# LunaJang/Metabuli_work

Hardware: AMD Instinct MI355X
Metric: reads/sec classified (150bp & 10kb) vs GTDB-scale DB at 1/2/4/8 MI355X (higher is better)
Workload: dtype u64

## Files before the change

### metabuli_work_amd/csrc/mtb_assign.hip

```cpp
#include <algorithm>
#include <vector>

#include "mtb_launch.h"
#include "mtb_stdsort.h"

namespace mtb {

struct Path {
    int start, end;
    float score;
    int hd, depth;
    uint32_t sm, em;
};

__device__ __forceinline__ void match_key(const mtb_match& m, uint64_t& hi, uint64_t& lo) {
    hi = ((uint64_t)m.species_id << 32) | ((uint64_t)info_frame(m.qinfo) << 29) | (info_pos(m.qinfo) & 0x1FFFFFFFu);
    lo = ((uint64_t)m.hamming << 56) | ((uint64_t)(m.dna_encoding & 0xFFFFFFu) << 32) | m.target_id;
}

__device__ __forceinline__ bool key_gt(uint64_t ah, uint64_t al, uint64_t bh, uint64_t bl) {
    return ah > bh || (ah == bh && al > bl);
}

constexpr int kSmallSeg = 512;
// ... 2011 lines not shown
        const uint32_t reh = M[p.sm].right_end_hamming;
        p.start = c.end + 1;
        p.hd = max(0, p.hd - ham_fields(reh, range, true));
        p.score = p.score - score_fields(reh, range, true) - (float)(ol % 3);
    }
}

__device__ __forceinline__ void trim_path_reh(Path& p, const Path& c, int ol, uint32_t rehS, uint32_t rehE) {
    const int range = ol / 3;
    if (p.start < c.start) {
        p.end = c.start - 1;
        p.hd = max(0, p.hd - ham_fields(rehE, range, false));
        p.score = p.score - score_fields(rehE, range, false) - (float)(ol % 3);
    } else {
        p.start = c.end + 1;
        p.hd = max(0, p.hd - ham_fields(rehS, range, true));
        p.score = p.score - score_fields(rehS, range, true) - (float)(ol % 3);
    }
}

__device__ float combine_serial(const mtb_match* __restrict__ M, Path* Ps, long nP, Path* Cs) {
    stdsort::sort(Ps, Ps + nP, [](const Path& a, const Path& b) {
        if (a.score != b.score) return a.score > b.score;
        if (a.hd != b.hd) return a.hd < b.hd;
        return a.start > b.start;
    });
    long nC = 0;
    float score = 0.0f;
    for (long pi = 0; pi < nP; pi++) {
        if (nC == 0) {
            Cs[nC++] = Ps[pi];
            score += Ps[pi].score;
            continue;
        }
        bool overlapped = false;
        for (long j = 0; j < nC; j++) {
            Path& p = Ps[pi];
            const Path c = Cs[j];
            if ((p.end < c.start) || (c.end < p.start)) continue;
            const int ol = min(p.end, c.end) - max(p.start, c.start) + 1;
            if (ol == p.end - p.start + 1) { overlapped = true; break; }
            if (ol < 24) {
                trim_path(M, p, c, ol);
                continue;
            }
            overlapped = true;
            break;
        }
        if (!overlapped) {
            Cs[nC++] = Ps[pi];
            score += Ps[pi].score;
        }
    }
    return score;
}

__device__ __forceinline__ void species_score(float score, int readLength, const AssignCfg& cfg, float* spScore,
                                              uint8_t* spKeep, uint64_t s) {
    score = score / (float)readLength;
    score = (1.0f < score) ? 1.0f : score;
    spScore[s] = score;
    spKeep[s] = !(score < cfg.minScore);
}

constexpr int kWaveCombineMin = 24;
constexpr int kWaveCombineMax = 1024;

__global__ void __launch_bounds__(256) k_combine_paths(const mtb_match* __restrict__ M, const uint64_t* __restrict__ sStart,
                                                       uint64_t nS, const uint64_t* __restrict__ runGroup,
                                                       const uint64_t* __restrict__ gStart,
                                                       const uint32_t* __restrict__ pathCnt,
                                                       const uint32_t* __restrict__ qlen, AssignCfg cfg,
                                                       Path* __restrict__ P, Path* __restrict__ C,
                                                       float* __restrict__ spScore, uint8_t* __restrict__ spKeep,
                                                       uint64_t* __restrict__ waveList, uint32_t* __restrict__ waveCount) {
    const uint64_t s = (uint64_t)blockIdx.x * blockDim.x + threadIdx.x;
    if (s >= nS) return;
    const uint64_t ss = sStart[s], se = sStart[s + 1];
    uint64_t w = ss;
    for (uint64_t g = runGroup[s]; gStart[g] < se; g++) {
        const uint64_t src = gStart[g];
        const uint32_t cnt = pathCnt[g];
        if (src != w)
            for (uint32_t k = 0; k < cnt; k++) P[w + k] = P[src + k];
        w += cnt;
    }
    if (w == ss) { spKeep[s] = 0; return; }
    const long nP = (long)(w - ss);
    if (!cfg.generic && nP > kWaveCombineMin && nP <= kWaveCombineMax) {
        waveList[atomicAdd(waveCount, 1u)] = ((uint64_t)nP << 32) | s;
        return;
    }
    const int readLength = (int)qlen[info_seq(M[ss].qinfo) - 1];
    species_score(combine_serial(M, P + ss, nP, C + ss), readLength, cfg, spScore, spKeep, s);
}

__global__ void __launch_bounds__(64) k_combine_wave(const mtb_match* __restrict__ M, const uint64_t* __restrict__ sStart,
                                                     const uint64_t* __restrict__ waveList,
                                                     const uint32_t* __restrict__ qlen, AssignCfg cfg,
                                                     Path* __restrict__ P, Path* __restrict__ C,
                                                     float* __restrict__ spScore, uint8_t* __restrict__ spKeep,
                                                     unsigned long long* __restrict__ stats,
                                                     const uint64_t* __restrict__ order) {
    __shared__ uint64_t kbuf[2 * kWaveCombineMax];
    uint64_t* kh = kbuf;
    uint64_t* kl = kbuf + kWaveCombineMax;
    __shared__ uint16_t qrs[kWaveCombineMax], qre[kWaveCombineMax];
    const uint64_t e = waveList[order ? order[blockIdx.x] : blockIdx.x];
    const uint64_t s = (uint32_t)e;
    const int nP = (int)(e >> 32);
    const uint64_t ss = sStart[s];
    const Path* Ps = P + ss;
    const int lane = threadIdx.x;
    const int readLength = (int)qlen[info_seq(M[ss].qinfo) - 1];
    int p2 = 2;
    while (p2 < nP) p2 <<= 1;
    for (int i = lane; i < p2; i += 64) {
        if (i < nP) {
            const Path p = Ps[i];
            kh[i] = ((uint64_t)(~__float_as_uint(p.score)) << 32) | (uint32_t)p.hd;
            kl[i] = ((uint64_t)(~(uint32_t)p.start) << 32) | (uint32_t)i;
        } else {
            kh[i] = ~0ull;
            kl[i] = ~0ull;
        }
    }
    __syncthreads();
    for (int k = 2; k <= p2; k <<= 1) {
        for (int j = k >> 1; j > 0; j >>= 1) {
            for (int t = lane; t < (p2 >> 1); t += 64) {
                const int i = ((t & ~(j - 1)) << 1) | (t & (j - 1));
                const int ixj = i + j;
                const bool up = (i & k) == 0;
                const uint64_t ah = kh[i], al = kl[i], bh = kh[ixj], bl = kl[ixj];
                if (key_gt(ah, al, bh, bl) == up) {
                    kh[i] = bh; kl[i] = bl; kh[ixj] = ah; kl[ixj] = al;
                }
            }
            __syncthreads();
        }
    }
    bool tie = false;
    for (int i = lane; i + 1 < nP; i += 64) {
        if (kh[i] != kh[i + 1] || (kl[i] >> 32) != (kl[i + 1] >> 32)) continue;
        const Path a = Ps[(uint32_t)kl[i]], b = Ps[(uint32_t)kl[i + 1]];
        tie |= a.end != b.end || M[a.sm].right_end_hamming != M[b.sm].right_end_hamming ||
               M[a.em].right_end_hamming != M[b.em].right_end_hamming;
    }
    struct EmuKey {
        float score;
        int hd, start;
        uint32_t idx;
    };
    static_assert(sizeof(EmuKey) * kWaveCombineMax == sizeof(uint64_t) * 2 * kWaveCombineMax, "emulation keys fit");
    EmuKey* K = reinterpret_cast<EmuKey*>(kbuf);
    const bool emulate = __syncthreads_or(tie || cfg.emulateAll);
    if (emulate) {
        if (lane == 0) atomicAdd(&stats[1], 1ull);
        for (int i = lane; i < nP; i += 64) {
            const Path q = Ps[i];
            K[i] = EmuKey{q.score, q.hd, q.start, (uint32_t)i};
        }
        __syncthreads();
        if (lane == 0)
            stdsort::sort(K, K + nP, [](const EmuKey& a, const EmuKey& b) {
                if (a.score != b.score) return a.score > b.score;
                if (a.hd != b.hd) return a.hd < b.hd;
                return a.start > b.start;
            });
        __syncthreads();
    }
    constexpr int kPerLane = kWaveCombineMax / 64;
    uint32_t src[kPerLane];
#pragma unroll
    for (int t = 0; t < kPerLane; t++) {
        const int i = lane + 64 * t;
        src[t] = i < nP ? (emulate ? K[i].idx : (uint32_t)kl[i]) : 0u;
    }
    __syncthreads();
    int* qs = reinterpret_cast<int*>(kh);
    int* qe = qs + kWaveCombineMax;
    float* qsc = reinterpret_cast<float*>(kl);
    int* qhd = reinterpret_cast<int*>(kl) + kWaveCombineMax;
#pragma unroll
    for (int t = 0; t < kPerLane; t++) {
        const int i = lane + 64 * t;
        if (i < nP) {
            const Path q = Ps[src[t]];
            qs[i] = q.start; qe[i] = q.end; qsc[i] = q.score; qhd[i] = q.hd;
            qrs[i] = M[q.sm].right_end_hamming;
            qre[i] = M[q.em].right_end_hamming;
        }
    }
    __syncthreads();
    constexpr int kSlots = kWaveCombineMax / 64;
    int rs[kSlots], re[kSlots];
#pragma unroll
    for (int t = 0; t < kSlots; t++) { rs[t] = 0; re[t] = -1; }
    float score = 0.0f;
    int nC = 0;
    for (int pi = 0; pi < nP; pi++) {
        Path p;
        p.start = qs[pi]; p.end = qe[pi]; p.score = qsc[pi]; p.hd = qhd[pi]; p.sm = 0; p.em = 0;
        const uint32_t rehS = qrs[pi], rehE = qre[pi];
        p.depth = 0;
        bool keep = true;
#pragma unroll
        for (int t = 0; t < kSlots; t++) {
            if (!keep || 64 * t >= nC) break;
            unsigned long long m = __ballot(64 * t + lane < nC && !(p.end < rs[t] || re[t] < p.start));
            while (keep && m) {
                const int l = __ffsll((long long)m) - 1;
                m &= m - 1;
                Path c;
                c.start = __shfl(rs[t], l, 64);
                c.end = __shfl(re[t], l, 64);
                if ((p.end < c.start) || (c.end < p.start)) continue;
                const int ol = min(p.end, c.end) - max(p.start, c.start) + 1;
                if (ol == p.end - p.start + 1) { keep = false; break; }
                if (ol < 24) { trim_path_reh(p, c, ol, rehS, rehE); continue; }
                keep = false;
            }
        }
        if (keep) {
#pragma unroll
            for (int t = 0; t < kSlots; t++)
                if (t == (nC >> 6) && lane == (nC & 63)) { rs[t] = p.start; re[t] = p.end; }
            nC++;
            score += p.score;
        }
    }
    if (lane == 0) species_score(score, readLength, cfg, spScore, spKeep, s);
}

__device__ long filter_redundant_serial(const mtb_match* __restrict__ M, uint64_t bestFirst, uint64_t bestSecond,
                                        uint64_t bestGroup, const uint64_t* __restrict__ gStart,
                                        uint32_t dnaShift, const TaxView& tax, mtb_taxcnt* __restrict__ tc) {
    uint32_t fc[6], fin[6], head[6];
    const mtb_match* B = M + bestFirst;
    int nf = 0;
    for (uint64_t g = bestGroup; nf < 6 && gStart[g] < bestSecond; g++) {
        fc[nf] = (uint32_t)(gStart[g] - bestFirst);
        fin[nf] = (uint32_t)(gStart[g + 1] - bestFirst);
        nf++;
    }
#pragma unroll
    for (int f = 0; f < 6; f++) head[f] = (f < nf) ? info_pos(B[fc[f]].qinfo) / dnaShift : 0xFFFFFFFFu;
    constexpr int kRegTc = 4;
    int32_t rt[kRegTc];
    uint32_t rc[kRegTc];
    long nTc = 0;
    while (true) {
        uint32_t qmin = 0xFFFFFFFFu;
#pragma unroll
        for (int f = 0; f < 6; f++) qmin = min(qmin, head[f]);
        if (qmin == 0xFFFFFFFFu) break;
        uint32_t minH = 256;
        int32_t t = 0;
#pragma unroll
        for (int f = 0; f < 6; f++) {
            while (head[f] == qmin) {
                const mtb_match& x = B[fc[f]];
                const uint32_t h = x.hamming;
                if (h < minH) { minH = h; t = (int32_t)x.target_id; }
                else if (h == minH) t = tax.lca(t, (int32_t)x.target_id);
                fc[f]++;
                head[f] = fc[f] < fin[f] ? info_pos(B[fc[f]].qinfo) / dnaShift : 0xFFFFFFFFu;
            }
        }
        long e = -1;
#pragma unroll
        for (int k = 0; k < kRegTc; k++)
            if (k < nTc && rt[k] == t) e = k;
        if (e >= 0) {
#pragma unroll
            for (int k = 0; k < kRegTc; k++)
                if (k == e) rc[k]++;
            continue;
        }
        if (nTc < kRegTc) {
#pragma unroll
            for (int k = 0; k < kRegTc; k++)
                if (k == nTc) { rt[k] = t; rc[k] = 1; }
            nTc++;
            continue;
        }
        e = kRegTc;
        while (e < nTc && tc[e].tax_id != t) e++;
        if (e == nTc) { tc[nTc].tax_id = t; tc[nTc].count = 0; nTc++; }
        tc[e].count++;
    }
#pragma unroll
    for (int k = 0; k < kRegTc; k++)
        if (k < nTc) { tc[k].tax_id = rt[k]; tc[k].count = rc[k]; }
    for (long a = 1; a < nTc; a++) {
        mtb_taxcnt v = tc[a];
        long b = a;
        while (b > 0 && tc[b - 1].tax_id > v.tax_id) { tc[b] = tc[b - 1]; b--; }
        tc[b] = v;
    }
    return nTc;
}

__device__ void classify_tail(mtb_result& res, const mtb_taxcnt* __restrict__ tc, long nTc, float spTotal,
                              int32_t bestTax, int readLength, const AssignCfg& cfg, const TaxView& tax,
                              Clade* __restrict__ cl, long clCap) {
    res.taxcnt_offset = (uint32_t)0;
    res.taxcnt_len = (uint32_t)nTc;
    res.is_classified = 1;
    res.score = spTotal;
    if (spTotal < cfg.minSpScore) {
        res.classification = tax.exists(bestTax) ? tax.spParent[tax.nodeOf[bestTax]] : 0;
        return;
    }
    if (cfg.em) {
        res.classification = bestTax;
        return;
    }
    const int32_t spT = bestTax;
    long nCl = 0;
    auto findOrAdd = [&](int32_t t) -> long {
        for (long z = 0; z < nCl; z++)
            if (cl[z].tax == t) return z;
        if (nCl >= clCap) return -1;
        cl[nCl].tax = t;
        cl[nCl].parentTax = 0;
        cl[nCl].count = 0;
        cl[nCl].removed = 0;
        return nCl++;
    };
    for (long e = 0; e < nTc; e++) {
        const uint32_t c = tc[e].count;
        int node = tax.nodeOf[tc[e].tax_id];
        int32_t t = tax.nodeTax[node];
        long z = findOrAdd(t);
        if (z < 0) break;
        cl[z].count += c;
        int guard = 0;
        while (t != spT && guard++ < 64) {
            const int pnode = tax.parent[node];
            const int32_t pt = tax.nodeTax[pnode];
            cl[z].parentTax = pt;
            long pz = findOrAdd(pt);
            if (pz < 0) break;
            cl[pz].count += c;
            node = pnode;
            t = pt;
            z = pz;
        }
    }
    if (cfg.accessionLevel == 2) {
        for (long z = 0; z < nCl; z++)
            if (cl[z].tax != spT && (tax.flags[tax.nodeOf[cl[z].tax]] & 2u)) cl[z].removed = 1;
    }
    const uint32_t thr = (uint32_t)((readLength - 1) / cfg.denominator);
    int32_t cur = spT;
    for (int step = 0; step < 64; step++) {
        uint32_t maxCnt = thr;
        long nBest = 0, best = -1, nChild = 0;
        for (long z = 0; z < nCl; z++) {
            if (cl[z].tax == spT || cl[z].removed || cl[z].parentTax != cur) continue;
            nChild++;
            const uint32_t cc = cl[z].count;
            if (cc > maxCnt) { maxCnt = cc; best = z; nBest = 1; }
            else if (cc == maxCnt) { if (nBest == 0) best = z; nBest++; }
        }
        if (nChild == 0 || nBest != 1) break;
        cur = cl[best].tax;
    }
    res.classification = cur;
}

__device__ __forceinline__ mtb_result empty_result(int readLength) {
    mtb_result res;
    res.classification = 0;
    res.score = 0.0f;
    res.hamming_dist = 0;
    res.query_length = (uint32_t)readLength;
    res.taxcnt_offset = (uint32_t)0;
    res.taxcnt_len = 0;
    res.is_classified = 0;
    for (int k = 0; k < 7; k++) res.pad[k] = 0;
    return res;
}

__global__ void __launch_bounds__(256) k_choose_taxon(const mtb_match* __restrict__ M, const uint64_t* __restrict__ mOff,
                                                      const uint32_t* __restrict__ qlen, uint32_t nReads,
                                                      const uint64_t* __restrict__ runOff,
                                                      const uint64_t* __restrict__ sStart,
                                                      const uint64_t* __restrict__ runGroup,
                                                      const uint64_t* __restrict__ gStart,
                                                      const float* __restrict__ spScore,
                                                      const uint8_t* __restrict__ spKeep, AssignCfg cfg, TaxView tax,
                                                      Clade* __restrict__ cladeP,
                                                      uint32_t cladePerMatch, mtb_taxcnt* __restrict__ tcP,
                                                      mtb_result* __restrict__ results) {
    const uint32_t r = blockIdx.x * blockDim.x + threadIdx.x;
    if (r >= nReads) return;
    const uint64_t base = mOff[r];
    const long n = (long)(mOff[r + 1] - base);
    const int readLength = (int)qlen[r];
    mtb_result res = empty_result(readLength);
    if (n == 0) { results[r] = res; return; }

    const uint64_t s0 = runOff[r], s1 = runOff[r + 1];
    long meaningful = 0;
    float bestSpScore = 0.0f;
    uint64_t bestFirst = 0, bestSecond = 0, bestRun = 0;
    for (uint64_t s = s0; s < s1; s++) {
        if (!spKeep[s]) continue;
        const float score = spScore[s];
        if (score > 0.f) meaningful++;
        if (score > bestSpScore) { bestSpScore = score; bestFirst = sStart[s]; bestSecond = sStart[s + 1]; bestRun = s; }
    }

    float spTotal = 0.0f;
    int32_t bestTax = 0;
    bool isLCA = false;
    if (meaningful > 0) {
        const float thr = bestSpScore * cfg.tieRatio;
        long cnt = 0;
        int lcaNode = -1;
        for (uint64_t s = s0; s < s1; s++) {
            if (!spKeep[s]) continue;
            if (spScore[s] >= thr) {
                cnt++;
                spTotal += spScore[s];
                const int32_t t = (int32_t)M[sStart[s]].species_id;
                if (cnt == 1) bestTax = t;
                if (tax.exists(t)) lcaNode = lcaNode < 0 ? tax.nodeOf[t] : tax.lca_node(lcaNode, tax.nodeOf[t]);
            }
        }
        if (cnt > 1) {
            isLCA = true;
            bestTax = lcaNode >= 0 ? tax.nodeTax[lcaNode] : 0;
            spTotal = spTotal / (float)cnt;
        }
    }
    if (spTotal == 0 || spTotal < cfg.minScore) {
        res.score = spTotal;
        results[r] = res;
        return;
    }
    if (isLCA) {
        res.is_classified = 1;
        res.classification = bestTax;
        res.score = spTotal;
        results[r] = res;
        return;
    }
    mtb_taxcnt* tc = tcP + base;
    const long nTc = filter_redundant_serial(M, bestFirst, bestSecond, runGroup[bestRun], gStart, (uint32_t)cfg.dnaShift, tax, tc);
    classify_tail(res, tc, nTc, spTotal, bestTax, readLength, cfg, tax, cladeP + base * cladePerMatch,
                  n * (long)cladePerMatch);
    results[r] = res;
}

constexpr int kWavePerReadMatches = 256;
constexpr int kQuotLds = 4096;
constexpr int kTcHash = 256;

__device__ __forceinline__ float wave_max_f(float x) {
#pragma unroll
    for (int d = 32; d > 0; d >>= 1) x = fmaxf(x, __shfl_xor(x, d, 64));
    return x;
}
__device__ __forceinline__ long wave_sum_l(long x) {
#pragma unroll
    for (int d = 32; d > 0; d >>= 1) x += __shfl_xor(x, d, 64);
    return x;
}

__global__ void __launch_bounds__(64) k_choose_taxon_wave(const mtb_match* __restrict__ M, const uint64_t* __restrict__ mOff,
                                                          const uint32_t* __restrict__ qlen, uint32_t nReads,
                                                          const uint64_t* __restrict__ runOff,
                                                          const uint64_t* __restrict__ sStart,
                                                          const uint64_t* __restrict__ runGroup,
                                                          const uint64_t* __restrict__ gStart,
                                                          const float* __restrict__ spScore,
                                                          const uint8_t* __restrict__ spKeep, AssignCfg cfg,
                                                          TaxView tax, Clade* __restrict__ cladeP,
                                                          uint32_t cladePerMatch, mtb_taxcnt* __restrict__ tcP,
                                                          mtb_result* __restrict__ results,
                                                          const uint64_t* __restrict__ order) {
    __shared__ uint32_t qw[kQuotLds];
    __shared__ int32_t hk[kTcHash];
    __shared__ uint32_t hc[kTcHash];
    __shared__ int sFlag;
    if (blockIdx.x >= nReads) return;
    const uint32_t r = order ? (uint32_t)order[blockIdx.x] : blockIdx.x;
    const int lane = threadIdx.x;
    const uint64_t base = mOff[r];
    const long n = (long)(mOff[r + 1] - base);
    const int readLength = (int)qlen[r];
    mtb_result res = empty_result(readLength);
    if (n == 0) {
        if (lane == 0) results[r] = res;
        return;
    }
    const uint64_t s0 = runOff[r], s1 = runOff[r + 1];
    long meaningful = 0;
    float bestSpScore = 0.0f;
    for (uint64_t s = s0 + lane; s < s1; s += 64) {
        if (!spKeep[s]) continue;
        const float score = spScore[s];
        meaningful += score > 0.f;
        bestSpScore = fmaxf(bestSpScore, score);
    }
    meaningful = wave_sum_l(meaningful);
    bestSpScore = wave_max_f(bestSpScore);
    float spTotal = 0.0f;
    int32_t bestTax = 0;
    bool isLCA = false;
    uint64_t bestFirst = 0, bestSecond = 0, bestRun = 0;
    if (meaningful > 0) {
        for (uint64_t c = s0; c < s1; c += 64) {
            const uint64_t s = c + lane;
            const bool hit = s < s1 && spKeep[s] && spScore[s] == bestSpScore;
            const unsigned long long m = __ballot(hit);
            if (m) {
                const uint64_t sb = c + (uint64_t)(__ffsll((long long)m) - 1);
                bestRun = sb;
                bestFirst = sStart[sb];
                bestSecond = sStart[sb + 1];
                break;
            }
        }
        const float thr = bestSpScore * cfg.tieRatio;
        long cnt = 0;
        int lcaNode = -1;
        for (uint64_t c = s0; c < s1; c += 64) {
            const uint64_t s = c + lane;
            const bool in = s < s1 && spKeep[s] && spScore[s] >= thr;
            const float sc = in ? spScore[s] : 0.0f;
            const int32_t sp = in ? (int32_t)M[sStart[s]].species_id : 0;
            unsigned long long m = __ballot(in);
            while (m) {
                const int b = __ffsll((long long)m) - 1;
                m &= m - 1;
                const float v = __shfl(sc, b, 64);
                const int32_t t = __shfl(sp, b, 64);
                cnt++;
                spTotal += v;
                if (cnt == 1) bestTax = t;
                if (tax.exists(t)) lcaNode = lcaNode < 0 ? tax.nodeOf[t] : tax.lca_node(lcaNode, tax.nodeOf[t]);
            }
        }
        if (cnt > 1) {
            isLCA = true;
            bestTax = lcaNode >= 0 ? tax.nodeTax[lcaNode] : 0;
            spTotal = spTotal / (float)cnt;
        }
    }
    if (spTotal == 0 || spTotal < cfg.minScore || isLCA) {
        if (lane == 0) {
            res.score = spTotal;
            if (isLCA && !(spTotal == 0 || spTotal < cfg.minScore)) {
                res.is_classified = 1;
                res.classification = bestTax;
            }
            results[r] = res;
        }
        return;
    }
    mtb_taxcnt* tc = tcP + base;
    const uint32_t dnaShift = (uint32_t)cfg.dnaShift;
    const long maxQ = (readLength + 3) / (long)dnaShift;
    const long nb = (long)(bestSecond - bestFirst);
    const mtb_match* B = M + bestFirst;
    long nTc = -1;
    if (tax.maxTax < 0xFFFFFF) {
        for (int k = lane; k < kTcHash; k += 64) { hk[k] = 0; hc[k] = 0; }
        if (lane == 0) sFlag = 0;
        for (long q0 = 0; q0 <= maxQ; q0 += kQuotLds) {
            const long q1 = min(maxQ + 1, q0 + (long)kQuotLds);
            for (long q = q0 + lane; q < q1; q += 64) qw[q - q0] = 0xFFFFFFFFu;
            __syncthreads();
            for (long i = lane; i < nb; i += 64) {
                const uint32_t q = info_pos(B[i].qinfo) / dnaShift;
                if (q > (uint32_t)maxQ || B[i].hamming > 254u) { sFlag = 1; continue; }
                if ((long)q < q0 || (long)q >= q1) continue;
                atomicMin(&qw[q - q0], (uint32_t)B[i].hamming << 24 | 0xFFFFFFu);
            }
            __syncthreads();
            if (sFlag) break;
            for (long i = lane; i < nb; i += 64) {
                const uint32_t q = info_pos(B[i].qinfo) / dnaShift;
                if ((long)q < q0 || (long)q >= q1) continue;
                const uint32_t h = (uint32_t)B[i].hamming << 24;
                uint32_t old = qw[q - q0];
                if ((old & 0xFF000000u) != h) continue;
                const int32_t t = (int32_t)B[i].target_id;
                while (true) {
                    const uint32_t cur = old & 0xFFFFFFu;
                    const uint32_t nv = h | (uint32_t)(cur == 0xFFFFFFu ? t : tax.lca((int32_t)cur, t));
                    if (nv == old) break;
                    const uint32_t prev = atomicCAS(&qw[q - q0], old, nv);
                    if (prev == old) break;
                    old = prev;
                }
            }
            __syncthreads();
            for (long q = q0 + lane; q < q1; q += 64) {
                const uint32_t wq = qw[q - q0];
                const int32_t t = wq == 0xFFFFFFFFu ? 0 : (int32_t)(wq & 0xFFFFFFu);
                if (t == 0) continue;
                uint32_t h = ((uint32_t)t * 2654435761u) & (kTcHash - 1);
                int probes = 0;
                while (true) {
                    const int32_t prev = atomicCAS(&hk[h], 0, t);
                    if (prev == 0 || prev == t) { atomicAdd(&hc[h], 1u); break; }
                    h = (h + 1) & (kTcHash - 1);
                    if (++probes == kTcHash) { sFlag = 1; break; }
                }
            }
            __syncthreads();
            if (sFlag) break;
        }
        if (!sFlag) {
            long at = 0;
            for (int k0 = 0; k0 < kTcHash; k0 += 64) {
                const int k = k0 + lane;
                const bool v = hk[k] != 0;
                const unsigned long long m = __ballot(v);
                if (v) {
                    const long p = at + (long)__popcll(m & ((1ull << lane) - 1));
                    tc[p].tax_id = hk[k];
                    tc[p].count = hc[k];
                }
                at += (long)__popcll(m);
            }
            nTc = at;
        }
    }
    if (lane != 0) return;
    if (nTc < 0) {
        nTc = filter_redundant_serial(M, bestFirst, bestSecond, runGroup[bestRun], gStart, dnaShift, tax, tc);
    } else {
        for (long a = 1; a < nTc; a++) {
            mtb_taxcnt v = tc[a];
            long b = a;
            while (b > 0 && tc[b - 1].tax_id > v.tax_id) { tc[b] = tc[b - 1]; b--; }
            tc[b] = v;
        }
    }
    classify_tail(res, tc, nTc, spTotal, bestTax, readLength, cfg, tax, cladeP + base * cladePerMatch,
                  n * (long)cladePerMatch);
    results[r] = res;
}

constexpr int kGroupLanes = 16;
constexpr int kGroupQ = 128;
constexpr int kGroupHash = 64;

__device__ __forceinline__ float group_max_f(float x) {
#pragma unroll
    for (int d = kGroupLanes / 2; d > 0; d >>= 1) x = fmaxf(x, __shfl_xor(x, d, kGroupLanes));
    return x;
}
__device__ __forceinline__ long group_sum_l(long x) {
#pragma unroll
    for (int d = kGroupLanes / 2; d > 0; d >>= 1) x += __shfl_xor(x, d, kGroupLanes);
    return x;
}

__device__ __forceinline__ void group_lds_order() {
    __builtin_amdgcn_fence(__ATOMIC_RELEASE, "wavefront");
    __builtin_amdgcn_wave_barrier();
    __builtin_amdgcn_fence(__ATOMIC_ACQUIRE, "wavefront");
}

__global__ void __launch_bounds__(256) k_choose_taxon_group(const mtb_match* __restrict__ M,
                                                            const uint64_t* __restrict__ mOff,
                                                            const uint32_t* __restrict__ qlen, uint32_t nReads,
                                                            const uint64_t* __restrict__ runOff,
                                                            const uint64_t* __restrict__ sStart,
                                                            const uint64_t* __restrict__ runGroup,
                                                            const uint64_t* __restrict__ gStart,
                                                            const float* __restrict__ spScore,
                                                            const uint8_t* __restrict__ spKeep, AssignCfg cfg,
                                                            TaxView tax, Clade* __restrict__ cladeP,
                                                            uint32_t cladePerMatch, mtb_taxcnt* __restrict__ tcP,
                                                            mtb_result* __restrict__ results) {
    constexpr int kGroups = 256 / kGroupLanes;
    __shared__ uint32_t qw[kGroups][kGroupQ];
    __shared__ int32_t hk[kGroups][kGroupHash];
    __shared__ uint32_t hc[kGroups][kGroupHash];
    __shared__ int gFlag[kGroups];
    const int g = threadIdx.x / kGroupLanes, gl = threadIdx.x % kGroupLanes;
    const int gLane0 = (threadIdx.x & 63) & ~(kGroupLanes - 1);
    const uint32_t r = blockIdx.x * kGroups + g;
    const bool valid = r < nReads;
    const uint64_t base = valid ? mOff[r] : 0;
    const long n = valid ? (long)(mOff[r + 1] - base) : 0;
    const int readLength = valid ? (int)qlen[r] : 0;
    mtb_result res = empty_result(readLength);
    float spTotal = 0.0f;
    int32_t bestTax = 0;
    bool isLCA = false, filter = false;
    uint64_t bestFirst = 0, bestSecond = 0, bestRun = 0;
    if (n > 0) {
        const uint64_t s0 = runOff[r], s1 = runOff[r + 1];
        long meaningful = 0;
        float bestSpScore = 0.0f;
        for (uint64_t s = s0 + gl; s < s1; s += kGroupLanes) {
            if (!spKeep[s]) continue;
            const float score = spScore[s];
            meaningful += score > 0.f;
            bestSpScore = fmaxf(bestSpScore, score);
        }
        meaningful = group_sum_l(meaningful);
        bestSpScore = group_max_f(bestSpScore);
        if (meaningful > 0) {
            for (uint64_t c = s0; c < s1; c += kGroupLanes) {
                const uint64_t s = c + gl;
                const bool hit = s < s1 && spKeep[s] && spScore[s] == bestSpScore;
                const uint32_t m = (uint32_t)(__ballot(hit) >> gLane0) & 0xFFFFu;
                if (m) {
                    const uint64_t sb = c + (uint64_t)(__ffs((int)m) - 1);
                    bestRun = sb;
                bestFirst = sStart[sb];
                    bestSecond = sStart[sb + 1];
                    break;
                }
            }
            const float thr = bestSpScore * cfg.tieRatio;
            long cnt = 0;
            int lcaNode = -1;
            for (uint64_t c = s0; c < s1; c += kGroupLanes) {
                const uint64_t s = c + gl;
                const bool in = s < s1 && spKeep[s] && spScore[s] >= thr;
                const float sc = in ? spScore[s] : 0.0f;
                const int32_t sp = in ? (int32_t)M[sStart[s]].species_id : 0;
                uint32_t m = (uint32_t)(__ballot(in) >> gLane0) & 0xFFFFu;
                while (m) {
                    const int b = __ffs((int)m) - 1;
                    m &= m - 1;
                    const float v = __shfl(sc, b, kGroupLanes);
                    const int32_t t = __shfl(sp, b, kGroupLanes);
                    cnt++;
                    spTotal += v;
                    if (cnt == 1) bestTax = t;
                    if (tax.exists(t)) lcaNode = lcaNode < 0 ? tax.nodeOf[t] : tax.lca_node(lcaNode, tax.nodeOf[t]);
                }
            }
            if (cnt > 1) {
                isLCA = true;
                bestTax = lcaNode >= 0 ? tax.nodeTax[lcaNode] : 0;
                spTotal = spTotal / (float)cnt;
            }
        }
        filter = !(spTotal == 0 || spTotal < cfg.minScore || isLCA);
    }
    const uint32_t dnaShift = (uint32_t)cfg.dnaShift;
    const long maxQ = (readLength + 3) / (long)dnaShift;
    const long nb = (long)(bestSecond - bestFirst);
    const mtb_match* B = M + bestFirst;
    const bool lds = filter && maxQ < kGroupQ && tax.maxTax < 0xFFFFFF;
    if (lds) {
        for (long q = gl; q <= maxQ; q += kGroupLanes) qw[g][q] = 0xFFFFFFFFu;
        for (int k = gl; k < kGroupHash; k += kGroupLanes) {
            hk[g][k] = 0;
            hc[g][k] = 0;
        }
        if (gl == 0) gFlag[g] = 0;
    }
    group_lds_order();
    if (lds) {
        for (long i = gl; i < nb; i += kGroupLanes) {
            const uint32_t q = info_pos(B[i].qinfo) / dnaShift;
            if (q > (uint32_t)maxQ || B[i].hamming > 254u) {
                gFlag[g] = 1;
                continue;
            }
            atomicMin(&qw[g][q], (uint32_t)B[i].hamming << 24 | 0xFFFFFFu);
        }
    }
    group_lds_order();
    const bool ok = lds && !gFlag[g];
    if (ok) {
        for (long i = gl; i < nb; i += kGroupLanes) {
            const uint32_t q = info_pos(B[i].qinfo) / dnaShift;
            const uint32_t h = (uint32_t)B[i].hamming << 24;
            uint32_t old = qw[g][q];
            if ((old & 0xFF000000u) != h) continue;
            const int32_t t = (int32_t)B[i].target_id;
            while (true) {
                const uint32_t cur = old & 0xFFFFFFu;
                const uint32_t nv = h | (uint32_t)(cur == 0xFFFFFFu ? t : tax.lca((int32_t)cur, t));
                if (nv == old) break;
                const uint32_t prev = atomicCAS(&qw[g][q], old, nv);
                if (prev == old) break;
                old = prev;
            }
        }
    }
    group_lds_order();
    if (ok) {
        for (long q = gl; q <= maxQ; q += kGroupLanes) {
            const uint32_t wq = qw[g][q];
            const int32_t t = wq == 0xFFFFFFFFu ? 0 : (int32_t)(wq & 0xFFFFFFu);
            if (t == 0) continue;
            uint32_t h = ((uint32_t)t * 2654435761u) & (kGroupHash - 1);
            int probes = 0;
            while (true) {
                const int32_t prev = atomicCAS(&hk[g][h], 0, t);
                if (prev == 0 || prev == t) {
                    atomicAdd(&hc[g][h], 1u);
                    break;
                }
                h = (h + 1) & (kGroupHash - 1);
                if (++probes == kGroupHash) {
                    gFlag[g] = 1;
                    break;
                }
            }
        }
    }
    group_lds_order();
    mtb_taxcnt* tc = tcP + base;
    long nTc = -1;
    const bool packed = ok && !gFlag[g];
    if (packed) {
        static_assert(2 * kGroupHash <= kGroupQ, "the packed taxa fit the quotient table");
        long at = 0;
        for (int k0 = 0; k0 < kGroupHash; k0 += kGroupLanes) {
            const int k = k0 + gl;
            const bool v = hk[g][k] != 0;
            const uint32_t m = (uint32_t)(__ballot(v) >> gLane0) & 0xFFFFu;
            if (v) {
                const long p = at + (long)__popc(m & ((1u << gl) - 1));
                qw[g][2 * p] = (uint32_t)hk[g][k];
                qw[g][2 * p + 1] = hc[g][k];
            }
            at += (long)__popc(m);
        }
        nTc = at;
    }
    group_lds_order();
    if (packed) {
        for (long e = gl; e < nTc; e += kGroupLanes) {
            const int32_t t = (int32_t)qw[g][2 * e];
            long at = 0;
            for (long j = 0; j < nTc; j++) at += (int32_t)qw[g][2 * j] < t;
            tc[at].tax_id = t;
            tc[at].count = qw[g][2 * e + 1];
        }
    }
    if (gl != 0 || !valid) return;
    if (!filter) {
        res.score = spTotal;
        if (isLCA && n > 0 && !(spTotal == 0 || spTotal < cfg.minScore)) {
            res.is_classified = 1;
            res.classification = bestTax;
        }
        results[r] = res;
        return;
    }
    if (nTc < 0) nTc = filter_redundant_serial(M, bestFirst, bestSecond, runGroup[bestRun], gStart, dnaShift, tax, tc);
    classify_tail(res, tc, nTc, spTotal, bestTax, readLength, cfg, tax, cladeP + base * cladePerMatch,
                  n * (long)cladePerMatch);
    results[r] = res;
}

__global__ void k_wave_size_keys(const uint64_t* __restrict__ waveList, uint32_t n, uint64_t* __restrict__ keys) {
    const uint32_t i = blockIdx.x * blockDim.x + threadIdx.x;
    if (i < n) keys[i] = (uint64_t)(kWaveCombineMax - (uint32_t)(waveList[i] >> 32));
}
__global__ void k_read_size_keys(const uint64_t* __restrict__ mOff, uint32_t n, uint64_t* __restrict__ keys) {
    const uint32_t i = blockIdx.x * blockDim.x + threadIdx.x;
    if (i < n) keys[i] = 0xFFFFFFull - min<uint64_t>(mOff[i + 1] - mOff[i], 0xFFFFFFull);
}

static const uint64_t* longest_first(uint32_t n, int bits, const AssignScratch& s, hipStream_t st) {
    bool inB = false;
    radix_sort_pairs(s.ordKA, s.ordVA, s.ordKB, s.ordVB, n, 0, bits, false, true, s.radixCounts, s.radixOffs,
                     s.scanTmp, &inB, st);
    return inB ? s.ordVB : s.ordVA;
}

void launch_assign(const mtb_match* matches, const uint64_t* mOff, const uint32_t* qlen, uint32_t nReads, uint64_t nM, const AssignArgs& a, const TaxDevice& t, const AssignScratch& s,
                   mtb_taxcnt* tcPool, mtb_result* results, unsigned long long* devStats, uint64_t* hostStats,
                   hipStream_t st) {
    for (int i = 0; i < 4; i++) hostStats[i] = 0;
    if (nReads == 0) return;
    AssignCfg cfg{a.kmerFormat, a.dnaShift, a.maxCodonShift, a.denominator, a.minConsCnt, a.minConsCntEuk,
                  a.accessionLevel, a.minScore, a.minSpScore, a.tieRatio, a.generic, a.emulateAll, a.em};
    TaxView tv{t.nodeOf, t.nodeTax, t.parent, t.depth, t.flags, t.spParent, t.maxTax};
    exclusive_scan_u32(s.grpCnt, nReads, s.grpOff, s.scanTmp, st);
    exclusive_scan_u32(s.runCnt, nReads, s.runOff, s.scanTmp, st);
    if (nM) {
        launch_run_starts(s.runFlag, mOff, s.grpOff, s.runOff, nReads, s.gStart, s.sStart, s.runGroup, st);
        uint64_t cnt[2] = {0, 0};
        hipMemcpyAsync(&cnt[0], s.grpOff + nReads, sizeof(uint64_t), hipMemcpyDeviceToHost, st);
        hipMemcpyAsync(&cnt[1], s.runOff + nReads, sizeof(uint64_t), hipMemcpyDeviceToHost, st);
        hipStreamSynchronize(st);
        hostStats[0] = cnt[0];
        hostStats[2] = cnt[1];
        if (cnt[0]) {
            k_group_keys<<<(unsigned)((cnt[0] + 255) / 256), 256, 0, st>>>(
                s.gStart, cnt[0], s.ordKA, s.ordVA, s.pathCnt,
                prune_min_matches(a.minConsCnt, a.minConsCntEuk, a.maxCodonShift));
            bool inB = false;
            const uint64_t heavy = radix_sort_pairs(s.ordKA, s.ordVA, s.ordKB, s.ordVB, cnt[0], 32, 40, true, false,
                                                    s.radixCounts, s.radixOffs, s.scanTmp, &inB, st);
            hostStats[1] = heavy;
            if (heavy) {
                const bool waves = !a.generic && a.bigGroups && nM >= kBigGroup;
                if (waves) hipMemsetAsync(s.waveCount, 0, sizeof(uint32_t), st);
                const char* nl = getenv("MTB_PATHS_NOLDS");
                const bool noLds = nl && atoi(nl) == 4;
                const char* la = getenv("MTB_K6_LOOKAHEAD");
                const bool look = !la || atoi(la) != 0;
#define MTB_PATHS(L, W, A)                                                                                          \
    k_match_paths<L, W, A><<<(unsigned)((heavy + 63) / 64), 64, 0, st>>>(                                              \
        matches, s.gStart, inB ? s.ordKB : s.ordKA, heavy, cfg, tv, (Path*)s.local, (Path*)s.paths, s.conn,         \
        s.pathCnt, waves ? s.waveList : nullptr, s.waveCount)
                if (noLds && look) MTB_PATHS(false, 4, true);
                else if (noLds) MTB_PATHS(false, 4, false);
                else if (look) MTB_PATHS(true, 1, true);
                else MTB_PATHS(true, 1, false);
#undef MTB_PATHS
                if (waves) {
                    uint32_t nBig = 0;
                    hipMemcpyAsync(&nBig, s.waveCount, sizeof(uint32_t), hipMemcpyDeviceToHost, st);
                    hipStreamSynchronize(st);
                    if (nBig && look)
                        k_match_paths_wave<true><<<nBig, 64, 0, st>>>(matches, s.gStart, s.waveList, cfg, tv, (Path*)s.local,
                                                                      (Path*)s.paths, s.conn, s.pathCnt);
                    else if (nBig)
                        k_match_paths_wave<false><<<nBig, 64, 0, st>>>(matches, s.gStart, s.waveList, cfg, tv, (Path*)s.local,
                                                                       (Path*)s.paths, s.conn, s.pathCnt);
                }
            }
        }
        if (cnt[1]) {
            hipMemsetAsync(s.waveCount, 0, sizeof(uint32_t), st);
            k_combine_paths<<<(unsigned)((cnt[1] + 255) / 256), 256, 0, st>>>(
                matches, s.sStart, cnt[1], s.runGroup, s.gStart, s.pathCnt, qlen, cfg, (Path*)s.paths, (Path*)s.comb,
                s.spScore, s.spKeep, s.waveList, s.waveCount);
            uint32_t nWave = 0;
            hipMemcpyAsync(&nWave, s.waveCount, sizeof(uint32_t), hipMemcpyDeviceToHost, st);
            hipStreamSynchronize(st);
            if (nWave) {
                k_wave_size_keys<<<(nWave + 255) / 256, 256, 0, st>>>(s.waveList, nWave, s.ordKA);
                const uint64_t* order = longest_first(nWave, 16, s, st);
                k_combine_wave<<<nWave, 64, 0, st>>>(matches, s.sStart, s.waveList, qlen, cfg, (Path*)s.paths,
                                                     (Path*)s.comb, s.spScore, s.spKeep, devStats, order);
            }
            hostStats[3] = nWave;
        }
    }
    const bool wave = a.waveTaxon >= 0 ? a.waveTaxon == 1 : (!a.generic && nM > (uint64_t)kWavePerReadMatches * nReads);
    const bool group = a.waveTaxon == 2 || (a.waveTaxon < 0 && !wave && !a.generic);
    if (group) {
        k_choose_taxon_group<<<(nReads + 15) / 16, 256, 0, st>>>(matches, mOff, qlen, nReads, s.runOff, s.sStart,
                                                                 s.runGroup, s.gStart, s.spScore, s.spKeep, cfg, tv,
                                                                 (Clade*)s.clade, s.cladePerMatch, tcPool, results);
    } else if (wave) {
        k_read_size_keys<<<(nReads + 255) / 256, 256, 0, st>>>(mOff, nReads, s.ordKA);
        const uint64_t* order = longest_first(nReads, 24, s, st);
        k_choose_taxon_wave<<<nReads, 64, 0, st>>>(matches, mOff, qlen, nReads, s.runOff, s.sStart, s.runGroup, s.gStart,
                                                   s.spScore, s.spKeep, cfg, tv, (Clade*)s.clade, s.cladePerMatch,
                                                   tcPool, results, order);
    } else {
        const unsigned ctT = nReads < 256u * 256u ? 64u : 256u;
        k_choose_taxon<<<(nReads + ctT - 1) / ctT, ctT, 0, st>>>(matches, mOff, qlen, nReads, s.runOff, s.sStart,
                                                             s.runGroup, s.gStart, s.spScore, s.spKeep, cfg, tv,
                                                             (Clade*)s.clade, s.cladePerMatch, tcPool, results);
    }
}

uint64_t path_bytes() { return sizeof(Path); }
uint64_t clade_bytes() { return sizeof(Clade); }

__global__ void k_compact_taxcnt(const mtb_taxcnt* __restrict__ pool, const uint64_t* __restrict__ mOff,
                                 mtb_result* __restrict__ results, const uint64_t* __restrict__ tcOff, uint32_t nReads,
                                 mtb_taxcnt* __restrict__ out) {
    uint32_t r = blockIdx.x * blockDim.x + threadIdx.x;
    if (r >= nReads) return;
    uint32_t len = results[r].taxcnt_len;
    uint64_t dst = tcOff[r];
    results[r].taxcnt_offset = (uint32_t)dst;
    for (uint32_t k = 0; k < len; k++) out[dst + k] = pool[mOff[r] + k];
}

__global__ void k_taxcnt_len(const mtb_result* __restrict__ results, uint32_t nReads, uint32_t* __restrict__ len) {
    uint32_t r = blockIdx.x * blockDim.x + threadIdx.x;
    if (r < nReads) len[r] = results[r].taxcnt_len;
}

void launch_taxcnt_len(const mtb_result* results, uint32_t nReads, uint32_t* len, hipStream_t s) {
    if (nReads) k_taxcnt_len<<<(nReads + 255) / 256, 256, 0, s>>>(results, nReads, len);
}
void launch_compact_taxcnt(const mtb_taxcnt* pool, const uint64_t* mOff, mtb_result* results, const uint64_t* tcOff,
                           uint32_t nReads, mtb_taxcnt* out, hipStream_t s) {
    if (nReads) k_compact_taxcnt<<<(nReads + 255) / 256, 256, 0, s>>>(pool, mOff, results, tcOff, nReads, out);
}

__global__ void k_chunk_totals(const uint32_t* __restrict__ cnt, uint32_t nChunks, uint32_t n,
                               uint32_t* __restrict__ tot) {
    const uint32_t r = blockIdx.x * blockDim.x + threadIdx.x;
    if (r >= n) return;
    uint32_t t = 0;
    for (uint32_t c = 0; c < nChunks; c++) t += cnt[(uint64_t)c * n + r];
    tot[r] = t;
}

__global__ void __launch_bounds__(256) k_regroup_chunks(const uint64_t* __restrict__ src, const uint32_t* __restrict__ cnt,
                                                        const uint64_t* __restrict__ srcOff, uint32_t nChunks, uint32_t n,
                                                        const uint64_t* __restrict__ mOff, uint64_t* __restrict__ dst) {
    const uint32_t r = blockIdx.x * 4 + threadIdx.x / 64;
    const uint32_t lane = threadIdx.x & 63;
    if (r >= n) return;
    uint64_t at = mOff[r] * 3;
    for (uint32_t c = 0; c < nChunks; c++) {
        const uint64_t k = (uint64_t)c * n + r;
        const uint64_t words = (uint64_t)cnt[k] * 3, from = srcOff[k] * 3;
        for (uint64_t w = lane; w < words; w += 64) dst[at + w] = src[from + w];
        at += words;
    }
}

void launch_regroup_chunks(const mtb_match* src, const uint32_t* cnt, uint32_t nChunks, uint32_t n, uint32_t* tot,
                           uint64_t* srcOff, uint64_t* mOff, void* scanTmp, mtb_match* dst, hipStream_t s) {
    if (!n) return;
    k_chunk_totals<<<(n + 255) / 256, 256, 0, s>>>(cnt, nChunks, n, tot);
    exclusive_scan_u32(tot, n, mOff, scanTmp, s);
    exclusive_scan_u32(cnt, (uint64_t)nChunks * n, srcOff, scanTmp, s);
    k_regroup_chunks<<<(n + 3) / 4, 256, 0, s>>>((const uint64_t*)src, cnt, srcOff, nChunks, n, mOff, (uint64_t*)dst);
}

struct EmPair {
    int32_t sp;
    float sc;
};

__global__ void k_em_top(const mtb_match* __restrict__ M, const uint64_t* __restrict__ mOff, uint32_t n,
                         const uint64_t* __restrict__ runOff, const uint64_t* __restrict__ sStart,
                         const float* __restrict__ spScore, const uint8_t* __restrict__ spKeep,
                         const mtb_result* __restrict__ results, EmPair* __restrict__ scratch,
                         EmPair* __restrict__ maps, uint8_t* __restrict__ cnt) {
    const uint32_t r = blockIdx.x * blockDim.x + threadIdx.x;
    if (r >= n) return;
    cnt[r] = 0;
    if (!results[r].is_classified) return;
    const uint64_t s0 = runOff[r], s1 = runOff[r + 1];
    EmPair* v = scratch + s0;
    long k = 0;
    for (uint64_t s = s0; s < s1; s++)
        if (spKeep[s]) v[k++] = EmPair{(int32_t)M[sStart[s]].species_id, spScore[s]};
    stdsort::sort(v, v + k, [](const EmPair& a, const EmPair& b) { return a.sc > b.sc; });
    const long m = k < kEmTop ? k : kEmTop;
    for (long i = 0; i < m; i++) maps[(uint64_t)r * kEmTop + i] = EmPair{v[i].sp, v[i].sc * v[i].sc};
    cnt[r] = (uint8_t)m;
}

void launch_em_top(const mtb_match* M, const uint64_t* mOff, uint32_t n, const AssignScratch& s,
                   const mtb_result* results, void* scratch, void* maps, uint8_t* cnt, hipStream_t st) {
    if (!n) return;
    k_em_top<<<(n + 255) / 256, 256, 0, st>>>(M, mOff, n, s.runOff, s.sStart, s.spScore, s.spKeep, results,
                                              (EmPair*)scratch, (EmPair*)maps, cnt);
}

__global__ void k_em_pack(const EmPair* __restrict__ maps, const uint8_t* __restrict__ cnt,
                          const uint64_t* __restrict__ off, uint32_t n, mtb_em_map* __restrict__ out) {
    const uint32_t r = blockIdx.x * blockDim.x + threadIdx.x;
    if (r >= n) return;
    const uint64_t o = off[r];
    for (uint32_t k = 0; k < cnt[r]; k++) {
        const EmPair e = maps[(uint64_t)r * kEmTop + k];
        out[o + k] = mtb_em_map{r, e.sp, e.sc};
    }
}

__global__ void k_u8_to_u32(const uint8_t* __restrict__ in, uint32_t n, uint32_t* __restrict__ out) {
    const uint32_t i = blockIdx.x * blockDim.x + threadIdx.x;
    if (i < n) out[i] = in[i];
}

void launch_em_pack(const void* maps, const uint8_t* cnt, uint32_t n, uint32_t* cnt32, uint64_t* off, void* scanTmp,
                    mtb_em_map* out, hipStream_t s) {
    if (!n) return;
    k_u8_to_u32<<<(n + 255) / 256, 256, 0, s>>>(cnt, n, cnt32);
    exclusive_scan_u32(cnt32, n, off, scanTmp, s);
    k_em_pack<<<(n + 255) / 256, 256, 0, s>>>((const EmPair*)maps, cnt, off, n, out);
}

__global__ void k_species_kmers(const DbRec* __restrict__ db, uint64_t D, const int32_t* __restrict__ spOf,
                                uint32_t maxTax, uint32_t* __restrict__ cnt) {
    MTB_GRID_STRIDE(i, D) {
        const uint32_t t = db[i].tax;
        const int32_t sp = t <= maxTax ? spOf[t] : 0;
        if (sp > 0) atomicAdd(&cnt[sp], 1u);
    }
}

void launch_species_kmers(const DbRec* db, uint64_t D, const int32_t* spOf, uint32_t maxTax, uint32_t* cnt,
                          hipStream_t s) {
    if (D) k_species_kmers<<<stride_grid(D), 256, 0, s>>>(db, D, spOf, maxTax, cnt);
}

__global__ void k_em_estep(const float* __restrict__ score, const uint32_t* __restrict__ spIdx,
                           const uint64_t* __restrict__ qOff, uint64_t nQ, const uint64_t* __restrict__ pos,
                           const double* __restrict__ p, const double* __restrict__ lf, double* __restrict__ wS,
                           unsigned long long* __restrict__ qCount) {
    const uint64_t q = (uint64_t)blockIdx.x * blockDim.x + threadIdx.x;
    bool counted = false;
    if (q < nQ) {
        const uint64_t a = qOff[q], b = qOff[q + 1];
        double denom = 0.0;
        for (uint64_t j = a; j < b; j++) denom += (double)score[j] * p[spIdx[j]] * lf[spIdx[j]];
        counted = !(denom == 0.0);
        for (uint64_t j = a; j < b; j++)
            wS[pos[j]] = counted ? ((double)score[j] * p[spIdx[j]] * lf[spIdx[j]]) / denom : 0.0;
    }
    const int c = __syncthreads_count(counted);
    if (threadIdx.x == 0 && c) atomicAdd(qCount, (unsigned long long)c);
}

__global__ void k_em_slices(const double* __restrict__ wS, const uint64_t* __restrict__ sliceOff, uint64_t nSl,
                            double* __restrict__ part) {
    const uint64_t i = (uint64_t)blockIdx.x * blockDim.x + threadIdx.x;
    if (i >= nSl) return;
    double f = 0.0;
    for (uint64_t j = sliceOff[i]; j < sliceOff[i + 1]; j++) f += wS[j];
    part[i] = f;
}

__global__ void k_em_mstep(const double* __restrict__ part, const uint64_t* __restrict__ spSlice, uint32_t S,
                           const uint8_t* __restrict__ isTop, const unsigned long long* __restrict__ qCount,
                           const double* __restrict__ p, double* __restrict__ pNew, double* __restrict__ absd,
                           int afterTen) {
    const uint32_t i = blockIdx.x * blockDim.x + threadIdx.x;
    if (i >= S) return;
    double f = 0.0;
    for (uint64_t k = spSlice[i]; k < spSlice[i + 1]; k++) f += part[k];
    if (isTop[i]) {
        f /= (double)*qCount;
        absd[i] = fabs(f - p[i]);
        if (afterTen && f < 1e-5) f = 0.0;
    } else {
        absd[i] = 0.0;
    }
    pNew[i] = f;
}

__global__ void __launch_bounds__(256) k_em_delta(const double* __restrict__ absd, uint32_t S, double* __restrict__ out) {
    __shared__ double part[256];
    const uint32_t per = (S + 255) / 256, a = threadIdx.x * per, b = min(S, a + per);
    double d = 0.0;
    for (uint32_t i = a; i < b; i++) d += absd[i];
    part[threadIdx.x] = d;
    __syncthreads();
    if (threadIdx.x == 0) {
        double t = 0.0;
        for (int k = 0; k < 256; k++) t += part[k];
        *out = t;
    }
}

void launch_em_iteration(const float* score, const uint32_t* spIdx, const uint64_t* qOff, uint64_t nQ,
                         const uint64_t* pos, const double* p, const double* lf, double* wS,
                         unsigned long long* qCount, const uint64_t* sliceOff, uint64_t nSl, double* part,
// ... 92 lines not shown
```

Measured before the change: 35.45 million.

## Keep clade table, sorted taxon counts and match fields on-chip in group assign

The group-per-read assign kernel now runs the clade-walk classification tail against a small LDS table that reuses the hash arrays. It falls back to the global clade buffer only when that table overflows, and reads the sorted taxon-count list from LDS when it is small. It also holds the first few match records per lane in registers between the min-hamming and LCA-fold passes, and caches per-lane species keep/score values when a read has at most one lane-stride of runs. The aim is to cut repeated global memory traffic in the serial lane-0 tail and the match re-reads, at the cost of extra registers, an extra wave barrier and a possible rerun when the table overflows.

```diff
diff --git a/metabuli_work_amd/csrc/mtb_assign.hip b/metabuli_work_amd/csrc/mtb_assign.hip
--- a/metabuli_work_amd/csrc/mtb_assign.hip
+++ b/metabuli_work_amd/csrc/mtb_assign.hip
@@ -2337,48 +2337,89 @@
     return nTc;
 }
 
-__device__ void classify_tail(mtb_result& res, const mtb_taxcnt* __restrict__ tc, long nTc, float spTotal,
-                              int32_t bestTax, int readLength, const AssignCfg& cfg, const TaxView& tax,
-                              Clade* __restrict__ cl, long clCap) {
+constexpr int kCladeLds = 32;
+struct TcGlobal {
+    const mtb_taxcnt* __restrict__ tc;
+    __device__ __forceinline__ int32_t tax(long e) const { return tc[e].tax_id; }
+    __device__ __forceinline__ uint32_t count(long e) const { return tc[e].count; }
+};
+struct TcLds {
+    const uint32_t* w;
+    __device__ __forceinline__ int32_t tax(long e) const { return (int32_t)w[2 * e]; }
+    __device__ __forceinline__ uint32_t count(long e) const { return w[2 * e + 1]; }
+};
+struct CladeGlobal {
+    static constexpr bool kRerun = false;
+    Clade* __restrict__ cl;
+    long cap;
+    __device__ __forceinline__ long capacity() const { return cap; }
+    __device__ __forceinline__ int32_t& tax(long z) const { return cl[z].tax; }
+    __device__ __forceinline__ int32_t& parentTax(long z) const { return cl[z].parentTax; }
+    __device__ __forceinline__ uint32_t& count(long z) const { return cl[z].count; }
+    __device__ __forceinline__ int32_t& removed(long z) const { return cl[z].removed; }
+};
+struct CladeLds {
+    static constexpr bool kRerun = true;
+    int32_t* k;
+    uint32_t* c;
+    long cap;
+    __device__ __forceinline__ long capacity() const { return cap; }
+    __device__ __forceinline__ int32_t& tax(long z) const { return k[z]; }
+    __device__ __forceinline__ int32_t& parentTax(long z) const { return k[kCladeLds + z]; }
+    __device__ __forceinline__ uint32_t& count(long z) const { return c[z]; }
+    __device__ __forceinline__ uint32_t& removed(long z) const { return c[kCladeLds + z]; }
+};
+
+template <typename Tc, typename Cl>
+__device__ __forceinline__ bool classify_tail_on(mtb_result& res, const Tc& tc, long nTc, float spTotal, int32_t bestTax,
+                                                 int readLength, const AssignCfg& cfg, const TaxView& tax,
+                                                 const Cl& cl) {
     res.taxcnt_offset = (uint32_t)0;
     res.taxcnt_len = (uint32_t)nTc;
     res.is_classified = 1;
     res.score = spTotal;
     if (spTotal < cfg.minSpScore) {
         res.classification = tax.exists(bestTax) ? tax.spParent[tax.nodeOf[bestTax]] : 0;
-        return;
+        return true;
     }
     if (cfg.em) {
         res.classification = bestTax;
-        return;
+        return true;
     }
     const int32_t spT = bestTax;
+    const long clCap = cl.capacity();
     long nCl = 0;
     auto findOrAdd = [&](int32_t t) -> long {
         for (long z = 0; z < nCl; z++)
-            if (cl[z].tax == t) return z;
+            if (cl.tax(z) == t) return z;
         if (nCl >= clCap) return -1;
-        cl[nCl].tax = t;
-        cl[nCl].parentTax = 0;
-        cl[nCl].count = 0;
-        cl[nCl].removed = 0;
+        cl.tax(nCl) = t;
+        cl.parentTax(nCl) = 0;
+        cl.count(nCl) = 0;
+        cl.removed(nCl) = 0;
         return nCl++;
     };
     for (long e = 0; e < nTc; e++) {
-        const uint32_t c = tc[e].count;
-        int node = tax.nodeOf[tc[e].tax_id];
+        const uint32_t c = tc.count(e);
+        int node = tax.nodeOf[tc.tax(e)];
         int32_t t = tax.nodeTax[node];
         long z = findOrAdd(t);
-        if (z < 0) break;
-        cl[z].count += c;
+        if (z < 0) {
+            if (Cl::kRerun) return false;
+            break;
+        }
+        cl.count(z) += c;
         int guard = 0;
         while (t != spT && guard++ < 64) {
             const int pnode = tax.parent[node];
             const int32_t pt = tax.nodeTax[pnode];
-            cl[z].parentTax = pt;
+            cl.parentTax(z) = pt;
             long pz = findOrAdd(pt);
-            if (pz < 0) break;
-            cl[pz].count += c;
+            if (pz < 0) {
+                if (Cl::kRerun) return false;
+                break;
+            }
+            cl.count(pz) += c;
             node = pnode;
             t = pt;
             z = pz;
@@ -2386,7 +2427,7 @@
     }
     if (cfg.accessionLevel == 2) {
         for (long z = 0; z < nCl; z++)
-            if (cl[z].tax != spT && (tax.flags[tax.nodeOf[cl[z].tax]] & 2u)) cl[z].removed = 1;
+            if (cl.tax(z) != spT && (tax.flags[tax.nodeOf[cl.tax(z)]] & 2u)) cl.removed(z) = 1;
     }
     const uint32_t thr = (uint32_t)((readLength - 1) / cfg.denominator);
     int32_t cur = spT;
@@ -2394,16 +2435,23 @@
         uint32_t maxCnt = thr;
         long nBest = 0, best = -1, nChild = 0;
         for (long z = 0; z < nCl; z++) {
-            if (cl[z].tax == spT || cl[z].removed || cl[z].parentTax != cur) continue;
+            if (cl.tax(z) == spT || cl.removed(z) || cl.parentTax(z) != cur) continue;
             nChild++;
-            const uint32_t cc = cl[z].count;
+            const uint32_t cc = cl.count(z);
             if (cc > maxCnt) { maxCnt = cc; best = z; nBest = 1; }
             else if (cc == maxCnt) { if (nBest == 0) best = z; nBest++; }
         }
         if (nChild == 0 || nBest != 1) break;
-        cur = cl[best].tax;
+        cur = cl.tax(best);
     }
     res.classification = cur;
+    return true;
+}
+
+__device__ void classify_tail(mtb_result& res, const mtb_taxcnt* __restrict__ tc, long nTc, float spTotal,
+                              int32_t bestTax, int readLength, const AssignCfg& cfg, const TaxView& tax,
+                              Clade* __restrict__ cl, long clCap) {
+    classify_tail_on(res, TcGlobal{tc}, nTc, spTotal, bestTax, readLength, cfg, tax, CladeGlobal{cl, clCap});
 }
 
 __device__ __forceinline__ mtb_result empty_result(int readLength) {
@@ -2687,6 +2735,10 @@
 constexpr int kGroupLanes = 16;
 constexpr int kGroupQ = 128;
 constexpr int kGroupHash = 64;
+constexpr int kHeld = 6;
+constexpr int kTcLds = 32;
+static_assert(2 * kCladeLds <= kGroupHash, "the on-chip clade table fits the two hash arrays");
+static_assert(4 * kTcLds <= kGroupQ, "packed pairs and sorted list fit the quotient table");
 
 __device__ __forceinline__ float group_max_f(float x) {
 #pragma unroll
@@ -2736,11 +2788,17 @@
     uint64_t bestFirst = 0, bestSecond = 0, bestRun = 0;
     if (n > 0) {
         const uint64_t s0 = runOff[r], s1 = runOff[r + 1];
+        const bool one = s1 - s0 <= (uint64_t)kGroupLanes;
+        const bool mine = one && s0 + gl < s1;
+        const uint8_t keepMine = mine ? spKeep[s0 + gl] : (uint8_t)0;
+        const float scoreMine = mine ? spScore[s0 + gl] : 0.0f;
+        auto kept = [&](uint64_t s) -> bool { return one ? keepMine != 0 : spKeep[s] != 0; };
+        auto scoreOf = [&](uint64_t s) -> float { return one ? scoreMine : spScore[s]; };
         long meaningful = 0;
         float bestSpScore = 0.0f;
         for (uint64_t s = s0 + gl; s < s1; s += kGroupLanes) {
-            if (!spKeep[s]) continue;
-            const float score = spScore[s];
+            if (!kept(s)) continue;
+            const float score = scoreOf(s);
             meaningful += score > 0.f;
             bestSpScore = fmaxf(bestSpScore, score);
         }
@@ -2749,12 +2807,12 @@
         if (meaningful > 0) {
             for (uint64_t c = s0; c < s1; c += kGroupLanes) {
                 const uint64_t s = c + gl;
-                const bool hit = s < s1 && spKeep[s] && spScore[s] == bestSpScore;
+                const bool hit = s < s1 && kept(s) && scoreOf(s) == bestSpScore;
                 const uint32_t m = (uint32_t)(__ballot(hit) >> gLane0) & 0xFFFFu;
                 if (m) {
                     const uint64_t sb = c + (uint64_t)(__ffs((int)m) - 1);
                     bestRun = sb;
-                bestFirst = sStart[sb];
+                    bestFirst = sStart[sb];
                     bestSecond = sStart[sb + 1];
                     break;
                 }
@@ -2764,8 +2822,8 @@
             int lcaNode = -1;
             for (uint64_t c = s0; c < s1; c += kGroupLanes) {
                 const uint64_t s = c + gl;
-                const bool in = s < s1 && spKeep[s] && spScore[s] >= thr;
-                const float sc = in ? spScore[s] : 0.0f;
+                const bool in = s < s1 && kept(s) && scoreOf(s) >= thr;
+                const float sc = in ? scoreOf(s) : 0.0f;
                 const int32_t sp = in ? (int32_t)M[sStart[s]].species_id : 0;
                 uint32_t m = (uint32_t)(__ballot(in) >> gLane0) & 0xFFFFu;
                 while (m) {
@@ -2801,34 +2859,59 @@
         if (gl == 0) gFlag[g] = 0;
     }
     group_lds_order();
-    if (lds) {
-        for (long i = gl; i < nb; i += kGroupLanes) {
-            const uint32_t q = info_pos(B[i].qinfo) / dnaShift;
-            if (q > (uint32_t)maxQ || B[i].hamming > 254u) {
-                gFlag[g] = 1;
-                continue;
-            }
-            atomicMin(&qw[g][q], (uint32_t)B[i].hamming << 24 | 0xFFFFFFu);
-        }
+    uint32_t heldQ[kHeld];
+    int32_t heldT[kHeld];
+    auto minHamming = [&](uint32_t q, uint32_t ham) -> bool {
+        if (q > (uint32_t)maxQ || ham > 254u) {
+            gFlag[g] = 1;
+            return false;
+        }
+        atomicMin(&qw[g][q], ham << 24 | 0xFFFFFFu);
+        return true;
+    };
+    auto foldTaxon = [&](uint32_t q, uint32_t h, int32_t t) {
+        uint32_t old = qw[g][q];
+        if ((old & 0xFF000000u) != h) return;
+        while (true) {
+            const uint32_t cur = old & 0xFFFFFFu;
+            const uint32_t nv = h | (uint32_t)(cur == 0xFFFFFFu ? t : tax.lca((int32_t)cur, t));
+            if (nv == old) break;
+            const uint32_t prev = atomicCAS(&qw[g][q], old, nv);
+            if (prev == old) break;
+            old = prev;
+        }
+    };
+#pragma unroll
+    for (int k = 0; k < kHeld; k++) {
+        heldQ[k] = 0xFFFFFFFFu;
+        heldT[k] = 0;
+    }
+    if (lds && nb > 0) {
+        uint32_t ham[kHeld];
+#pragma unroll
+        for (int k = 0; k < kHeld; k++) {
+            const long i = min((long)(gl + k * kGroupLanes), nb - 1);
+            heldQ[k] = info_pos(B[i].qinfo);
+            ham[k] = B[i].hamming;
+            heldT[k] = (int32_t)B[i].target_id;
+        }
+#pragma unroll
+        for (int k = 0; k < kHeld; k++) {
+            const uint32_t q = heldQ[k] / dnaShift;
+            const bool have = gl + k * kGroupLanes < nb;
+            heldQ[k] = have && minHamming(q, ham[k]) ? ham[k] << 24 | q : 0xFFFFFFFFu;
+        }
+        for (long i = gl + kHeld * kGroupLanes; i < nb; i += kGroupLanes)
+            minHamming(info_pos(B[i].qinfo) / dnaShift, (uint32_t)B[i].hamming);
     }
     group_lds_order();
     const bool ok = lds && !gFlag[g];
     if (ok) {
-        for (long i = gl; i < nb; i += kGroupLanes) {
-            const uint32_t q = info_pos(B[i].qinfo) / dnaShift;
-            const uint32_t h = (uint32_t)B[i].hamming << 24;
-            uint32_t old = qw[g][q];
-            if ((old & 0xFF000000u) != h) continue;
-            const int32_t t = (int32_t)B[i].target_id;
-            while (true) {
-                const uint32_t cur = old & 0xFFFFFFu;
-                const uint32_t nv = h | (uint32_t)(cur == 0xFFFFFFu ? t : tax.lca((int32_t)cur, t));
-                if (nv == old) break;
-                const uint32_t prev = atomicCAS(&qw[g][q], old, nv);
-                if (prev == old) break;
-                old = prev;
-            }
-        }
+#pragma unroll
+        for (int k = 0; k < kHeld; k++)
+            if (heldQ[k] != 0xFFFFFFFFu) foldTaxon(heldQ[k] & 0xFFFFFFu, heldQ[k] & 0xFF000000u, heldT[k]);
+        for (long i = gl + kHeld * kGroupLanes; i < nb; i += kGroupLanes)
+            foldTaxon(info_pos(B[i].qinfo) / dnaShift, (uint32_t)B[i].hamming << 24, (int32_t)B[i].target_id);
     }
     group_lds_order();
     if (ok) {
@@ -2873,15 +2956,23 @@
         nTc = at;
     }
     group_lds_order();
+    const bool tcLds = packed && nTc <= kTcLds;
+    uint32_t* sorted = qw[g] + 2 * kTcLds;
     if (packed) {
         for (long e = gl; e < nTc; e += kGroupLanes) {
             const int32_t t = (int32_t)qw[g][2 * e];
+            const uint32_t c = qw[g][2 * e + 1];
             long at = 0;
             for (long j = 0; j < nTc; j++) at += (int32_t)qw[g][2 * j] < t;
             tc[at].tax_id = t;
-            tc[at].count = qw[g][2 * e + 1];
-        }
-    }
+            tc[at].count = c;
+            if (tcLds) {
+                sorted[2 * at] = (uint32_t)t;
+                sorted[2 * at + 1] = c;
+            }
+        }
+    }
+    group_lds_order();
     if (gl != 0 || !valid) return;
     if (!filter) {
         res.score = spTotal;
@@ -2893,8 +2984,12 @@
         return;
     }
     if (nTc < 0) nTc = filter_redundant_serial(M, bestFirst, bestSecond, runGroup[bestRun], gStart, dnaShift, tax, tc);
-    classify_tail(res, tc, nTc, spTotal, bestTax, readLength, cfg, tax, cladeP + base * cladePerMatch,
-                  n * (long)cladePerMatch);
+    const CladeLds cl{hk[g], hc[g], min((long)kCladeLds, n * (long)cladePerMatch)};
+    const bool done = tcLds ? classify_tail_on(res, TcLds{sorted}, nTc, spTotal, bestTax, readLength, cfg, tax, cl)
+                            : classify_tail_on(res, TcGlobal{tc}, nTc, spTotal, bestTax, readLength, cfg, tax, cl);
+    if (!done)
+        classify_tail(res, tc, nTc, spTotal, bestTax, readLength, cfg, tax, cladeP + base * cladePerMatch,
+                      n * (long)cladePerMatch);
     results[r] = res;
 }
 
```

Result: no change. 35.91 million, median of 6 (+1.3%).
